# Isaac-McPadden/Farkle_II

Measured on AMD Instinct MI355X. Metric: simulated games/sec (whole node) at k=2, fixed strategy-grid size, higher is better.
Workload: dtype int32; 1 GPU; BASELINE configs[1]: k=2, 64-strategy grid, 10^7 games per GPU per step, root_seed 42, counts-only tallies; k=2, root_seed=42, parallelism=shuffle-range split x1, device=AMD Radeon Graphics, arch=gfx950:sramecc+:xnack-, compute_units=256, clock_mhz=2400

## Files before the change

farkle_ii_amd/csrc/fk_device.h:

```cpp
#pragma once

#include <hip/hip_runtime.h>
#include <stdint.h>

namespace fk {

constexpr uint32_t SS_INIT_A = 0x43b0d7e5u, SS_MULT_A = 0x931e8875u;
constexpr uint32_t SS_INIT_B = 0x8b51f9ddu, SS_MULT_B = 0x58f38dedu;
constexpr uint32_t SS_MIX_L = 0xca01f9ddu, SS_MIX_R = 0x4973f715u;

__host__ __device__ constexpr uint32_t ss_hc(int c) {
    uint32_t h = SS_INIT_A;
    for (int i = 0; i < c; ++i) h *= SS_MULT_A;
    return h;
}

__host__ __device__ inline uint32_t ss_hashmix(uint32_t v, uint32_t &hc) {
    v ^= hc;
    hc *= SS_MULT_A;
    v *= hc;
    v ^= v >> 16;
    return v;
}

// ... 765 lines not shown
    r.turn_score = farkle ? 0 : (r.turn_score + rr.score50);
    const bool hot = !farkle & sp.has(SF_AUTO_HOT) & (r.dice == 6u);
    if (LEAN) r.cB += hot ? 0x10000u : 0u;
    else r.cE += hot ? 1u : 0u;
    const bool keep = should_continue50(sp, r.turn_score, (int32_t)r.dice, (r.cE & BE_HAS_SCORED) != 0u, final_round, stb50, r.score);
    const bool over = farkle | (!hot & !keep);
    const uint32_t ts = over ? (uint32_t)r.turn_score : 0u;
    r.cE |= (ts >= 10u) ? BE_HAS_SCORED : 0u;
    const uint32_t banked = (r.cE & BE_HAS_SCORED) ? ts : 0u;
    r.score += (int32_t)banked;
    if (LEAN) r.cE += banked;
    r.cB = (banked > (r.cB & 0xffffu)) ? ((r.cB & 0xffff0000u) | banked) : r.cB;
    overflow = (r.turn_score > 1310) | ((r.cA & 0xffffu) > 64000u) | ((r.cC >> 16) > 63000u) | ((r.cD >> 16) > 63000u);
    return over;
}

typedef uint64_t lanes_t;
__host__ __device__ inline lanes_t lanes(bool p) {
#if defined(__HIP_DEVICE_COMPILE__)
    return __builtin_amdgcn_ballot_w64(p);
#else
    return p ? ~0ull : 0ull;
#endif
}
__host__ __device__ inline bool in_lanes(lanes_t m) {
#if defined(__HIP_DEVICE_COMPILE__)
    return __builtin_amdgcn_inverse_ballot_w64(m);
#else
    return m != 0ull;
#endif
}

template <uint32_t MIXED>
__host__ __device__ inline lanes_t flag_lanes(const Strat50 &s, uint32_t uniform_bits, uint32_t f) {
    return (f & MIXED) ? lanes((s.bits & f) != 0u) : ((uniform_bits & f) != 0u ? ~0ull : 0ull);
}

__host__ __device__ inline uint32_t pk_max_u16(uint32_t a, uint32_t b) {
#if defined(__HIP_DEVICE_COMPILE__)
    typedef unsigned short u16x2 __attribute__((ext_vector_type(2)));
    return __builtin_bit_cast(uint32_t, __builtin_elementwise_max(__builtin_bit_cast(u16x2, a), __builtin_bit_cast(u16x2, b)));
#else
    const uint32_t al = a & 0xffffu, bl = b & 0xffffu, ah = a >> 16, bh = b >> 16;
    return (al > bl ? al : bl) | ((ah > bh ? ah : bh) << 16);
#endif
}

template <bool LEAN, uint32_t MIXED>
__host__ __device__ inline bool roll_back_end50_core(int32_t score50, uint32_t used, uint32_t inc_c, uint32_t inc_d, uint32_t n, const Strat50 &sp,
                                                     uint32_t uniform_bits, bool final_round, int32_t stb50, RollRegs &r, bool &overflow) {
    const bool farkle = score50 == 0;
    r.cA += 1u + (farkle ? 0x10000u : 0u);
    r.cC += inc_c;
    r.cD += inc_d;
    r.dice = (used == n) ? 6u : (n - used);
    r.turn_score = farkle ? 0 : (r.turn_score + score50);
    const lanes_t farkle_l = lanes(score50 == 0);
    const lanes_t hot_l = ~farkle_l & flag_lanes<MIXED>(sp, uniform_bits, SF_AUTO_HOT) & lanes(r.dice == 6u);
    const bool hot = in_lanes(hot_l);
    if (LEAN) r.cB += hot ? 0x10000u : 0u;
    else r.cE += hot ? 1u : 0u;
    const lanes_t fr = lanes(final_round), above = lanes(r.score + r.turn_score > stb50);
    const lanes_t stop = fr & above & ~flag_lanes<MIXED>(sp, uniform_bits, SF_RUN_UP);
    const lanes_t force = fr & ~above;
    const lanes_t entry = lanes((r.cE & BE_HAS_SCORED) == 0u) & lanes(r.turn_score < 10);
    const lanes_t cs = flag_lanes<MIXED>(sp, uniform_bits, SF_CONSIDER_SCORE), cd = flag_lanes<MIXED>(sp, uniform_bits, SF_CONSIDER_DICE);
    const lanes_t ws = cs & lanes(r.turn_score < sp.thr50), wd = cd & lanes((int32_t)r.dice > sp.dice_thr());
    const lanes_t both = cs & cd & ~flag_lanes<MIXED>(sp, uniform_bits, SF_REQUIRE_BOTH);
    const lanes_t keep = ~stop & (force | entry | ((ws | wd) & (~both | (ws & wd))));
    const lanes_t over_l = farkle_l | (~hot_l & ~keep);
    const bool over = in_lanes(over_l), bank = in_lanes(over_l & ~entry);
    const uint32_t banked = bank ? (uint32_t)r.turn_score : 0u;
    r.cE |= bank ? BE_HAS_SCORED : 0u;
    r.score += (int32_t)banked;
    if (LEAN) r.cE += banked;
    r.cB = pk_max_u16(r.cB, banked);
    overflow = roll_overflow50(r);
    return over;
}

template <bool LEAN, uint32_t MIXED = 0xffffu>
__host__ __device__ inline bool roll_back_end50(uint32_t e, uint32_t choice, uint32_t n, const Strat50 &sp, uint32_t uniform_bits, bool final_round,
                                                int32_t stb50, RollRegs &r, bool &overflow) {
    const uint32_t d5 = choice & 3u, d1 = (choice >> 2) & 3u;
    const int32_t score50 = (int32_t)(e & 63u) - (int32_t)d5 - 2 * (int32_t)d1;
    const uint32_t used = ((e >> 6) & 7u) - d5 - d1;
    return roll_back_end50_core<LEAN, MIXED>(score50, used, (d5 << 16) + ((choice >> DCH_ANY5_SHIFT) & 1u), (d1 << 16) + ((choice >> DCH_ANY1_SHIFT) & 1u), n,
                                             sp, uniform_bits, final_round, stb50, r, overflow);
}

template <bool LEAN, uint32_t MIXED = 0xffffu>
__host__ __device__ inline bool roll_back_end50w(uint32_t e, uint32_t x, uint32_t n, const Strat50 &sp, uint32_t uniform_bits, bool final_round,
                                                 int32_t stb50, RollRegs &r, bool &overflow) {
    const int32_t score50 = (int32_t)(e & 63u) - (int32_t)((x >> DW_POINTS_SHIFT) & 0xffu);
    const uint32_t used = ((e >> 6) & 7u) - (x >> DW_DICE_SHIFT);
    return roll_back_end50_core<LEAN, MIXED>(score50, used, x & DW_INC, (x >> DW_D1_SHIFT) & DW_INC, n, sp, uniform_bits, final_round, stb50, r, overflow);
}

struct Table2 {
    uint32_t seat, rounds, trigger, final_round, safety;
    int32_t score_to_beat;
};
struct Advance2 {
    bool ended, sw;
};
__host__ __device__ inline Advance2 advance2_table50(bool over, int32_t score, int32_t target50, uint32_t max_rounds, Table2 &t) {
    const bool fr = t.final_round != 0u;
    const bool trig = over & !fr & (score >= target50);
    const bool close = over & !fr & !trig & (t.seat != 0u);
    const bool last = close & (t.rounds >= max_rounds);
    const bool ended = last | (over & fr);
    t.rounds += (close & !last) ? 1u : 0u;
    t.safety = last ? 1u : t.safety;
    t.score_to_beat = trig ? score : t.score_to_beat;
    t.trigger = trig ? t.seat : t.trigger;
    t.final_round = (fr | trig) ? 1u : 0u;
    const bool sw = over & !ended;
    t.seat ^= sw ? 1u : 0u;
    return Advance2{ended, sw};
}

constexpr uint32_t LEAN_IDX_SHIFT = 18;
struct LeanCounters {
    uint32_t cA, cB, cC, cD, cE;
};
struct Finish2 {
    bool completed;
    uint32_t winner, widx;
    uint32_t m[10];
};

__host__ __device__ inline Finish2 finish2_50_decoded(const LeanCounters &s0, const LeanCounters &s1, uint32_t rounds, uint32_t final_round,
                                                      uint32_t max_rounds) {
    const LeanCounters *seats[2] = {&s0, &s1};
    uint32_t score[2], idx[2], farkles[2], rolls[2], highest[2], sf_uses[2], sf_dice[2], so_uses[2], so_dice[2], hot[2];
    for (int s = 0; s < 2; ++s) {
        const LeanCounters &r = *seats[s];
        score[s] = r.cE & 0xffffu, idx[s] = r.cE >> LEAN_IDX_SHIFT;
        rolls[s] = r.cA & 0xffffu, farkles[s] = r.cA >> 16;
        highest[s] = r.cB & 0xffffu, hot[s] = r.cB >> 16;
        sf_uses[s] = r.cC & 0xffffu, sf_dice[s] = r.cC >> 16;
        so_uses[s] = r.cD & 0xffffu, so_dice[s] = r.cD >> 16;
    }
    Finish2 f;
    f.completed = max_rounds != 0u && final_round != 0u;
    f.winner = score[1] > score[0] ? 1u : 0u;
    const uint32_t w = f.winner;
    f.widx = idx[w];
    f.m[0] = score[w] * 50u, f.m[1] = rounds, f.m[2] = farkles[w], f.m[3] = rolls[w], f.m[4] = highest[w] * 50u;
    f.m[5] = sf_uses[w], f.m[6] = sf_dice[w], f.m[7] = so_uses[w], f.m[8] = so_dice[w], f.m[9] = hot[w];
    return f;
}

__host__ __device__ inline Finish2 finish2_50(const LeanCounters &s0, const LeanCounters &s1, uint32_t rounds, uint32_t final_round,
                                              uint32_t max_rounds) {
    (void)max_rounds;
    const bool second = (s1.cE & 0xffffu) > (s0.cE & 0xffffu);
    const uint32_t a = second ? s1.cA : s0.cA, b = second ? s1.cB : s0.cB, c = second ? s1.cC : s0.cC, d = second ? s1.cD : s0.cD,
                   e = second ? s1.cE : s0.cE;
    Finish2 f;
    f.completed = final_round != 0u;
    f.winner = second ? 1u : 0u;
    f.widx = e >> LEAN_IDX_SHIFT;
    f.m[0] = (e & 0xffffu) * 50u, f.m[1] = rounds, f.m[2] = a >> 16, f.m[3] = a & 0xffffu, f.m[4] = (b & 0xffffu) * 50u;
    f.m[5] = c & 0xffffu, f.m[6] = c >> 16, f.m[7] = d & 0xffffu, f.m[8] = d >> 16, f.m[9] = b >> 16;
    return f;
}

}
```

farkle_ii_amd/csrc/fk_kernels.h:

```cpp
#pragma once

#include "../../include/farkle_hip.h"
#include "fk_device.h"

#include <hip/hip_runtime.h>

#include <type_traits>

using namespace fk;

namespace {

constexpr uint32_t HC_AFTER_6_WORDS = ss_hc(24);
constexpr uint32_t HC_AFTER_12_WORDS = ss_hc(48);
constexpr uint32_t HC_AFTER_14_WORDS = ss_hc(56);

enum : uint32_t { MODE_PERM = 0, MODE_LIST = 1, MODE_BLOCKS = 2 };

enum : uint32_t {
    F_LO0 = 0, F_LO1, F_HI0, F_HI1, F_INC_LO0, F_INC_LO1, F_INC_HI0, F_INC_HI1,
    F_BUF, F_SCORE, F_CA, F_CB, F_CC, F_CD, F_CE, F_SPX, F_SPY, NF
};
constexpr uint32_t CE_HAS_BUF_SHIFT = 17, CE_HAS_SCORED = 1u << 16, CE_HAS_BUF = 1u << CE_HAS_BUF_SHIFT;
static_assert(CE_HAS_SCORED == BE_HAS_SCORED, "fk_device.h's roll back end sets the flag in cE");
// ... 934 lines not shown
            if (PK2) {
                const uint32_t *r0 = reinterpret_cast<const uint32_t *>(rec);
                rng.lo = (uint64_t)r0[0] | ((uint64_t)r0[1] << 32);
                rng.hi = (uint64_t)r0[2] | ((uint64_t)r0[3] << 32);
                rng.buf = r0[4];
            } else {
                rng.lo = (uint64_t)L(F_LO0, s) | ((uint64_t)L(F_LO1, s) << 32);
                rng.hi = (uint64_t)L(F_HI0, s) | ((uint64_t)L(F_HI1, s) << 32);
                rng.buf = L(F_BUF, s);
            }
            rng.has_buf = (cE & CE_HAS_BUF) ? 1u : 0u;
            key = 4u * roll_counts_sequential<3>(rng, n, nullptr);
        }
        rolls_this_turn += 1u;
        int32_t dthr = PK2 ? ((int32_t)own_bits >> 16) : (int32_t)(int8_t)(own_bits & 0xffu);
        asm volatile("" : "+v"(dthr));
        const Strat50 sp{own_thr, (own_bits & (0xffu | MIXED)) | (a.uflags & (0xff00u & ~MIXED)), dthr};
        uint32_t entry;
        const uint32_t choice = discard_lookup50w(a.score_lut, reinterpret_cast<const uint32_t *>(a.discard_lut + DISCARD_LUT_KEYS), key, (int32_t)n, turn_score, sp, entry);
        RollRegs rg{cA, cB, cC, cD, cE, score, dice, turn_score};
        bool overflow;
        const bool over = roll_back_end50w<LEAN, MIXED>(entry, choice, n, sp, a.uflags & (0xff00u & ~MIXED), final_round != 0u, score_to_beat, rg, overflow);
        cA = rg.cA, cB = rg.cB, cC = rg.cC, cD = rg.cD, cE = rg.cE, score = rg.score, dice = rg.dice, turn_score = rg.turn_score;
        const uint32_t guard = roll_guards50(rolls_before, rg);
        if (guard != RG_NONE) {
            raise(guard == RG_ROLL_LIMIT ? FK_ERR_ROLL_LIMIT : FK_ERR_COUNTER_OVERFLOW);
            return;
        }
        cE = (cE & ~CE_HAS_BUF) | (rng.has_buf << CE_HAS_BUF_SHIFT);
        if (GS) {
            if (over) {
                uint4 *g = reinterpret_cast<uint4 *>(G(s));
                g[0] = make_uint4((uint32_t)rng.lo, (uint32_t)(rng.lo >> 32), (uint32_t)rng.hi, (uint32_t)(rng.hi >> 32));
                g[1] = make_uint4(rng.buf, (uint32_t)score, cA, (cB & 0xffffu) | (own_turns << 16));
                uint32_t *g2 = reinterpret_cast<uint32_t *>(g + 2);
                g2[0] = cC;
                g2[1] = cD;
                g2[2] = (cB >> 16) | (cE & (CE_HAS_SCORED | CE_HAS_BUF));
                advance(score);
                return;
            }
        }
        if (LEAN) {
            rec[0] = make_uint2((uint32_t)rng.lo, (uint32_t)(rng.lo >> 32));
            rec[1] = make_uint2((uint32_t)rng.hi, (uint32_t)(rng.hi >> 32));
            rec[2] = make_uint2(rng.buf, cA);
            rec[3] = make_uint2(cB, cC);
            rec[4] = make_uint2(cD, cE);
        } else {
            L(F_LO0, s) = (uint32_t)rng.lo;
            L(F_LO1, s) = (uint32_t)(rng.lo >> 32);
            L(F_HI0, s) = (uint32_t)rng.hi;
            L(F_HI1, s) = (uint32_t)(rng.hi >> 32);
            L(F_BUF, s) = rng.buf;
            L(F_SCORE, s) = (uint32_t)score;
            L(F_CA, s) = cA;
            L(F_CB, s) = cB;
            L(F_CC, s) = cC;
            L(F_CD, s) = cD;
            L(F_CE, s) = cE;
        }
        if (PK2) advance2(over, score);
        else if (!GS && over) advance(score);
    };

    constexpr bool FLAT2 = PK2 && !BLK;
    static_assert(CE_IDX_SHIFT == LEAN_IDX_SHIFT, "finish2_50 reads the strategy index of a lean record");
    enum : uint32_t { HO_LDS_TALLY = 1, HO_REC0 = 2, HO_RECS = 4, HO_GS_OUT = 8, HO_OV = 16, HO_SCHED = 32, HO_PERM = 64, HO_IDX_STATE = 128,
                      HO_FLAT = 256 };
    typedef uint32_t u32x2 __attribute__((ext_vector_type(2)));
    typedef __attribute__((address_space(1))) u32x4 global_u4_rw;
    typedef const __attribute__((address_space(1))) u32x2 global_u2;
    typedef __attribute__((address_space(1))) uint32_t global_u32;
    uint32_t ho_bits = 0, st_rec = 0, ho_max_rounds = a.max_rounds, ho_thr = a.batch_threshold;
    int32_t ho_beat50 = a.beat50;
    uint64_t st_base = 0, inc_base = 0, idx_base = 0, sched_base = 0, strat_base = 0, rec0_base = 0;
    if constexpr (FLAT2) {
        const bool idx_state = a.state_dw == STATE_DW;
        const bool flat = !a.no_flat && (idx_state || a.seat_idx != nullptr) && (uint64_t)a.n_games * (2u * STATE_DW * 4u) <= 0xffffffffull;
        ho_bits = (a.use_lds_tally ? HO_LDS_TALLY : 0u) | (a.rec0 ? HO_REC0 : 0u) | (a.recs ? HO_RECS : 0u) | (a.gs_out ? HO_GS_OUT : 0u) |
             (a.n_ov ? HO_OV : 0u) | (a.sched ? HO_SCHED : 0u) | (a.mode == MODE_PERM ? HO_PERM : 0u) | (idx_state ? HO_IDX_STATE : 0u) |
             (flat ? HO_FLAT : 0u);
        st_rec = a.state_dw * 4u;
        st_base = (uint64_t)(uintptr_t)a.state, inc_base = (uint64_t)(uintptr_t)a.inc, sched_base = (uint64_t)(uintptr_t)a.sched;
        idx_base = idx_state ? st_base + R_IDX * 4u : (uint64_t)(uintptr_t)a.seat_idx;
        strat_base = (uint64_t)(uintptr_t)a.strat, rec0_base = (uint64_t)(uintptr_t)a.rec0;
        asm volatile("" : "+s"(ho_bits), "+s"(st_rec), "+s"(ho_max_rounds), "+s"(ho_thr), "+s"(ho_beat50), "+s"(st_base), "+s"(inc_base), "+s"(idx_base),
                     "+s"(sched_base), "+s"(strat_base), "+s"(rec0_base));
    }
    auto ld1 = [](uint64_t base, uint32_t off) __attribute__((always_inline)) -> uint32_t { return *(const global_u32 *)(base + (uint64_t)off); };
    auto ld2 = [](uint64_t base, uint32_t off) __attribute__((always_inline)) -> u32x2 { return *(global_u2 *)(base + (uint64_t)off); };
    auto ld4 = [](uint64_t base, uint32_t off) __attribute__((always_inline)) -> u32x4 { return *(global_u4 *)(base + (uint64_t)off); };

    auto init_game2 = [&](uint32_t ticket) __attribute__((always_inline)) {
        uint32_t ho = ho_bits;
        asm volatile("" : "+s"(ho));
        uint32_t id = ticket, slot = ticket;
        uint32_t id_ld = 0;
        if (ho & HO_SCHED) {
            id_ld = ld1(sched_base, ticket * 4u);
        } else if (ho & HO_PERM) {
            const uint32_t sh = id / a.gps, g = id - sh * a.gps;
            slot = g * a.n_sh + sh;
        }
        const uint32_t soff = slot * (2u * st_rec);
        const u32x4 s0 = ld4(st_base, soff), s1 = ld4(st_base, soff + st_rec);
        const u32x4 inc = ld4(inc_base, slot * 32u);
        const uint32_t ioff = (ho & HO_IDX_STATE) ? soff : slot * 4u;
        const uint32_t w0 = ld1(idx_base, ioff), w1 = ld1(idx_base, ioff + ((ho & HO_IDX_STATE) ? st_rec : 0u));
        if (ho & HO_SCHED) id = id_ld;
        const uint32_t idx0 = (ho & HO_IDX_STATE) ? w0 : (w0 & 0xffffu), idx1 = (ho & HO_IDX_STATE) ? w1 : (w1 >> 16);
        u32x2 pk0 = ld2(strat_base, idx0 * 8u), pk1 = ld2(strat_base, idx1 * 8u);
        game_id = id;
        seed_slot = slot;
        max_rounds = ho_max_rounds;
        if (ho & HO_OV) {
            uint32_t lo = 0, hi = a.n_ov;
            while (lo < hi) {
                const uint32_t mid = (lo + hi) >> 1;
                if (a.ov[mid].game < id) lo = mid + 1u;
                else hi = mid;
            }
            if (lo < a.n_ov && a.ov[lo].game == id) max_rounds = a.ov[lo].max_rounds;
        }
        uint2 *r0 = reinterpret_cast<uint2 *>(lds + lane_base), *r1 = reinterpret_cast<uint2 *>(lds + SEAT_STRIDE + lane_base);
        r0[0] = make_uint2(s0.x, s0.y), r0[1] = make_uint2(s0.z, s0.w);
        r0[2] = make_uint2(0u, 0u), r0[3] = make_uint2(0u, 0u), r0[4] = make_uint2(0u, idx0 << CE_IDX_SHIFT);
        r1[0] = make_uint2(s1.x, s1.y), r1[1] = make_uint2(s1.z, s1.w);
        r1[2] = make_uint2(0u, 0u), r1[3] = make_uint2(0u, 0u), r1[4] = make_uint2(0u, idx1 << CE_IDX_SHIFT);
        pk0.y = (pk0.y & 0xff00u) | ((uint32_t)(int32_t)(int8_t)(pk0.y & 0xffu) << 16);
        pk1.y = (pk1.y & 0xff00u) | ((uint32_t)(int32_t)(int8_t)(pk1.y & 0xffu) << 16);
        pk_seat0 = make_uint2(pk0.x, pk0.y);
        pk_delta = make_uint2(pk0.x ^ pk1.x, pk0.y ^ pk1.y);
        seat = 0;
        final_round = 0;
        score_to_beat = ho_beat50;
        own_inc_lo = (uint64_t)inc.x | ((uint64_t)inc.y << 32);
        own_inc_hi = (uint64_t)inc.z | ((uint64_t)inc.w << 32);
        own_thr = (int32_t)pk0.x;
        own_bits = pk0.y;
        own_rec = lds_addr(lane_base);
        own_inc_at = inc_base + (uint64_t)(slot * 32u);
        dice = 6;
        turn_score = 0;
        rolls_this_turn = 0;
        const bool none = max_rounds == 0u;
        rounds = none ? 0u : 1u;
        st = none ? (uint32_t)ST_ENDED : (uint32_t)ST_ACTIVE;
    };

    auto finish_game2 = [&]() __attribute__((always_inline)) {
        uint32_t ho = ho_bits;
        asm volatile("" : "+s"(ho));
        const uint2 *r0 = reinterpret_cast<const uint2 *>(lds + lane_base), *r1 = reinterpret_cast<const uint2 *>(lds + SEAT_STRIDE + lane_base);
        const uint2 p2 = r0[2], p3 = r0[3], p4 = r0[4], q2 = r1[2], q3 = r1[3], q4 = r1[4];
        const LeanCounters c0{p2.y, p3.x, p3.y, p4.x, p4.y}, c1{q2.y, q3.x, q3.y, q4.x, q4.y};
        const Finish2 f = finish2_50(c0, c1, rounds, final_round, max_rounds);
        const uint32_t idx0 = c0.cE >> CE_IDX_SHIFT, idx1 = c1.cE >> CE_IDX_SHIFT, widx = f.widx;
        if (ho & HO_GS_OUT) {
            const uint32_t last = (max_rounds != 0u && own_rec != lds_addr(lane_base)) ? 1u : 0u;
            const uint32_t t0 = rounds + ((final_round != 0u && last == 0u) ? 1u : 0u), t1 = rounds;
            const uint2 p0 = r0[0], p1 = r0[1], q0 = r1[0], q1 = r1[1];
            const uint32_t soff = seed_slot * (2u * st_rec);
            global_u4_rw *g0 = (global_u4_rw *)(st_base + (uint64_t)soff), *g1 = (global_u4_rw *)(st_base + (uint64_t)(soff + st_rec));
            g0[0] = u32x4{p0.x, p0.y, p1.x, p1.y};
            g0[1] = u32x4{p2.x, c0.cE & 0xffffu, c0.cA, (c0.cB & 0xffffu) | (t0 << 16)};
            g0[2] = u32x4{c0.cC, c0.cD, (c0.cB >> 16) | (c0.cE & (CE_HAS_SCORED | CE_HAS_BUF)), idx0};
            g1[0] = u32x4{q0.x, q0.y, q1.x, q1.y};
            g1[1] = u32x4{q2.x, c1.cE & 0xffffu, c1.cA, (c1.cB & 0xffffu) | (t1 << 16)};
            g1[2] = u32x4{c1.cC, c1.cD, (c1.cB >> 16) | (c1.cE & (CE_HAS_SCORED | CE_HAS_BUF)), idx1};
        }
        if (ho & HO_LDS_TALLY) {
            if (!f.completed || !(ho & HO_PERM)) {
                const uint32_t col = f.completed ? 1u : 2u;
                atomicAdd(&tl[idx0 * LT_COLS + col], 1ull);
                atomicAdd(&tl[idx1 * LT_COLS + col], 1ull);
            }
            if (f.completed) {
                unsigned long long *t = tl + widx * LT_COLS;
                atomicAdd(&t[0], 1ull);
#pragma unroll
                for (int j = 0; j < 10; ++j) {
                    atomicAdd(&t[3 + j], (unsigned long long)f.m[j]);
                    atomicAdd(&t[13 + j], (unsigned long long)f.m[j] * f.m[j]);
                }
            }
        }
        if (ho & HO_REC0) {
            const uint32_t d0 = f.completed ? (widx | (f.winner << 24)) : REC_SAFETY;
            *(global_u32 *)(rec0_base + (uint64_t)(game_id * 4u)) = d0;
            if (ho & HO_RECS) {
                uint32_t m[10];
#pragma unroll
                for (int j = 0; j < 10; ++j) m[j] = f.completed ? f.m[j] : 0u;
                uint4 *r = reinterpret_cast<uint4 *>(a.recs + (size_t)game_id * REC_DW);
                r[0] = make_uint4(d0, m[0], rounds | (m[2] << 16), m[3] | (m[4] << 16));
                r[1] = make_uint4(m[5] | (m[6] << 16), m[7] | (m[8] << 16), m[9], 0u);
            }
        }
    };

#ifdef FK_COUNT_HANDOVER
    uint32_t cnt_handovers = 0, cnt_served = 0, cnt_trips = 0, cnt_waiting = 0, cnt_rolling = 0;
#endif

    auto handover = [&](uint64_t waiting, auto flat) {
        constexpr bool FLAT = decltype(flat)::value;
        const bool mine = (st == ST_FRESH || st == ST_ENDED);
        if (st == ST_ENDED) {
            if constexpr (FLAT) finish_game2();
            else finish_game();
        }
        const uint32_t n = (uint32_t)__popcll(waiting);
        const uint32_t avail = pool_end - pool_next;
        uint32_t new_base = 0, new_avail = 0;
        if (avail < n && !exhausted) {
            const uint32_t first = (uint32_t)__builtin_amdgcn_readfirstlane(__ffsll((long long)waiting) - 1);
            uint32_t base = 0;
            if (mine && lane_id() == first) base = atomicAdd(a.ticket, TICKET_CHUNK);
            base = (uint32_t)__builtin_amdgcn_readlane((int)base, (int)first);
            if (base >= a.n_games) {
                exhausted = 1;
            } else {
                new_base = base;
                new_avail = min(TICKET_CHUNK, a.n_games - base);
                if (new_avail < TICKET_CHUNK) exhausted = 1;
            }
        }
        if (mine) {
            const uint32_t rank = mbcnt(waiting);
            uint32_t ticket = 0xffffffffu;
            if (rank < avail) ticket = pool_next + rank;
            else if (rank - avail < new_avail) ticket = new_base + (rank - avail);
            if (ticket != 0xffffffffu) {
                if constexpr (FLAT) init_game2(ticket);
                else init_game(a.sched ? a.sched[ticket] : ticket, ticket);
            } else {
                st = ST_DONE;
            }
        }
        if (n <= avail) {
            pool_next += n;
        } else {
            const uint32_t used_new = min(n - avail, new_avail);
            pool_next = new_base + used_new;
            pool_end = new_base + new_avail;
        }
    };

    auto handover_due = [&](uint64_t waiting, uint64_t active) -> bool {
        return waiting && (!active || (uint32_t)__popcll(waiting) >= ho_thr || exhausted);
    };
    auto play = [&](auto flat) {
        while (true) {
            uint64_t waiting = __ballot(st == ST_FRESH || st == ST_ENDED);
            uint64_t active = __ballot(st == ST_ACTIVE);
            if (!(waiting | active)) break;
            if (handover_due(waiting, active)) {
#ifdef FK_COUNT_HANDOVER
                cnt_handovers += 1u, cnt_served += (uint32_t)__popcll(waiting);
#endif
                handover(waiting, flat);
                continue;
            }
            bool playing = st == ST_ACTIVE;
            do {
#ifdef FK_COUNT_HANDOVER
                cnt_trips += 1u, cnt_waiting += (uint32_t)__popcll(waiting), cnt_rolling += (uint32_t)__popcll(active);
#endif
                if (playing) roll_step();
                playing = st == ST_ACTIVE;
                waiting = __ballot(st == ST_ENDED);
                active = __ballot(playing);
            } while (active && !handover_due(waiting, active));
        }
    };
    if constexpr (FLAT2) {
        if (ho_bits & HO_FLAT) play(std::true_type{});
        else play(std::false_type{});
    } else {
        play(std::false_type{});
    }

    if (a.use_lds_tally) {
        __syncthreads();
        for (uint32_t i = tid; i < a.S * LT_COLS; i += BLOCK) {
            const unsigned long long v = tl[i];
            if (v == 0ull) continue;
            const uint32_t idx = i / LT_COLS, c = i - idx * LT_COLS;
            if (c == LT_COLS - 1u) continue;
            const uint32_t col = (c == 0u) ? 0u : (c == 1u) ? 2u : (c == 2u) ? 3u : (c < 13u) ? (c + 1u) : (c + 2u);
            atomicAdd(&a.tally[(size_t)idx * FK_TALLY_COLS + col], v);
        }
    }
#ifdef FK_COUNT_HANDOVER
    if (a.hcount && lane_id() == 0u) {
        const uint32_t c[6] = {cnt_handovers, cnt_served, cnt_trips, cnt_waiting, cnt_rolling, 1u};
        for (int i = 0; i < 6; ++i) atomicAdd(&a.hcount[i], (unsigned long long)c[i]);
    }
#endif
    clock_stamp(a.clk, 1u);
}

#include "fk_play_hc.h"

constexpr uint32_t LAG_WIN_BIT = 0x8000u;

__global__ __launch_bounds__(256) void fk_lag_values_kernel(const uint32_t *recs, const uint16_t *perm_T, uint32_t perm_slots, uint32_t S,
                                                            uint32_t k, uint32_t gps, uint32_t n_games, uint16_t *V) {
    const size_t t = (size_t)blockIdx.x * blockDim.x + threadIdx.x;
    if (t >= (size_t)n_games * k) return;
    const uint32_t id = (uint32_t)(t / k), seat = (uint32_t)(t - (size_t)id * k);
    const uint32_t sh = id / gps, g = id - sh * gps;
    const uint4 q0 = *reinterpret_cast<const uint4 *>(recs + (size_t)id * REC_DW);
    const bool won = !(q0.x & REC_SAFETY) && ((q0.x >> 24) & 0x7fu) == seat;
    const uint32_t idx = perm_at(perm_T, S, perm_slots, sh, g * k + seat);
    V[(size_t)sh * S + idx] = (uint16_t)((q0.z & 0x7fffu) | (won ? LAG_WIN_BIT : 0u));
}

__global__ __launch_bounds__(256) void fk_lag_sums_kernel(const uint16_t *V, uint32_t S, uint32_t valid_from, uint32_t first_row, uint32_t n_rows,
                                                          uint32_t rows_per_seg, const int32_t *lags, uint32_t n_lags, long long *out) {
    const uint32_t s = blockIdx.x * blockDim.x + threadIdx.x;
    if (s >= S) return;
    const uint32_t r0 = first_row + blockIdx.y * rows_per_seg, r1 = min(r0 + rows_per_seg, n_rows);
    for (uint32_t li = 0; li < n_lags; ++li) {
        const uint32_t lag = (uint32_t)lags[li];
        long long n = 0, wx = 0, wy = 0, wxy = 0, rx = 0, ry = 0, rxx = 0, ryy = 0, rxy = 0;
        for (uint32_t r = max(r0, valid_from + lag); r < r1; ++r) {
            const uint32_t later = V[(size_t)r * S + s], earlier = V[(size_t)(r - lag) * S + s];
            const long long a = earlier & 0x7fffu, b = later & 0x7fffu, wa = earlier >> 15, wb = later >> 15;
            n += 1;
            wx += wa, wy += wb, wxy += wa & wb;
            rx += a, ry += b, rxx += a * a, ryy += b * b, rxy += a * b;
        }
        if (n == 0) continue;
        unsigned long long *o = reinterpret_cast<unsigned long long *>(out) + ((size_t)s * n_lags + li) * FK_LAG_COLS;
        const long long v[FK_LAG_COLS] = {n, wx, wy, wx, wy, wxy, rx, ry, rxx, ryy, rxy};
#pragma unroll
        for (int c = 0; c < FK_LAG_COLS; ++c)
            if (v[c]) atomicAdd(&o[c], (unsigned long long)v[c]);
    }
}


__device__ inline uint32_t walk_slot(uint32_t id, uint32_t gps, uint32_t n_sh, bool perm_mode) {
    if (!perm_mode) return id;
    const uint32_t sh = id / gps, g = id - sh * gps;
    return g * n_sh + sh;
}

constexpr uint32_t REDUCE_BLOCK = 1024, RT_COLS = 22;

__global__ __launch_bounds__(REDUCE_BLOCK) void fk_tally_reduce_kernel(const uint32_t *rec0, const uint32_t *recs, uint32_t n_games, uint32_t gps, uint32_t k,
                                                                       uint32_t S, const uint16_t *perm_T, uint32_t perm_slots,
                                                                       uint32_t sh_offset, uint32_t spb, uint32_t n_sh,
                                                                       uint32_t parts_per_batch, uint32_t slice, uint32_t first_batch,
                                                                       unsigned long long *tally) {
    extern __shared__ unsigned long long rt[];
    const uint32_t b_local = blockIdx.x / parts_per_batch, part = blockIdx.x - b_local * parts_per_batch;
    const uint32_t batch = first_batch + b_local;
    const uint64_t g_lo = (uint64_t)batch * spb, g_hi = g_lo + spb;
    const uint32_t sh_lo = g_lo > sh_offset ? (uint32_t)(g_lo - sh_offset) : 0u;
    const uint32_t sh_hi = (uint32_t)min<uint64_t>(n_sh, g_hi > sh_offset ? g_hi - sh_offset : 0u);
    if (sh_hi <= sh_lo) return;
    const uint32_t games = (sh_hi - sh_lo) * gps, per_part = (games + parts_per_batch - 1u) / parts_per_batch;
    const uint32_t first = sh_lo * gps + part * per_part, last = min(first + per_part, sh_lo * gps + games);
    const uint32_t s_lo = blockIdx.y * slice, s_n = min(slice, S - s_lo);
    for (uint32_t i = threadIdx.x; i < s_n * RT_COLS; i += REDUCE_BLOCK) rt[i] = 0ull;
    __syncthreads();
    constexpr uint32_t U = 4;
    for (uint32_t base = first + threadIdx.x; base < last; base += U * REDUCE_BLOCK) {
        uint32_t d0[U];
        uint4 q0[U], q1[U];
        bool mine[U];
#pragma unroll
        for (uint32_t u = 0; u < U; ++u) {
            const uint32_t id = base + u * REDUCE_BLOCK;
            d0[u] = id < last ? rec0[id] : REC_SAFETY - 1u;
        }
#pragma unroll
        for (uint32_t u = 0; u < U; ++u) {
            const uint32_t id = base + u * REDUCE_BLOCK;
            mine[u] = id < last && !(d0[u] & REC_SAFETY) && ((d0[u] & 0xffffffu) - s_lo) < s_n;
            if (mine[u]) {
                const uint4 *r = reinterpret_cast<const uint4 *>(recs + (size_t)id * REC_DW);
                q0[u] = r[0];
                q1[u] = r[1];
            }
        }
#pragma unroll
        for (uint32_t u = 0; u < U; ++u) {
            const uint32_t id = base + u * REDUCE_BLOCK;
            if (id < last && (d0[u] & REC_SAFETY)) {
                const uint32_t sh = id / gps, g = id - sh * gps;
                for (uint32_t s = 0; s < k; ++s) {
                    const uint32_t idx = perm_at(perm_T, S, perm_slots, sh, g * k + s) - s_lo;
                    if (idx < s_n) atomicAdd(&rt[idx * RT_COLS + 1u], 1ull);
                }
            }
            if (!mine[u]) continue;
            const uint32_t idx = (d0[u] & 0xffffffu) - s_lo;
            const unsigned long long m[10] = {q0[u].y, q0[u].z & 0xffffu, q0[u].z >> 16, q0[u].w & 0xffffu, q0[u].w >> 16,
                                              q1[u].x & 0xffffu, q1[u].x >> 16, q1[u].y & 0xffffu, q1[u].y >> 16, q1[u].z};
            unsigned long long *t = rt + idx * RT_COLS;
            atomicAdd(&t[0], 1ull);
#pragma unroll
            for (int j = 0; j < 10; ++j) {
                if (m[j]) {
                    atomicAdd(&t[2 + j], m[j]);
                    atomicAdd(&t[12 + j], m[j] * m[j]);
                }
            }
        }
    }
    __syncthreads();
    unsigned long long *out = tally + ((size_t)batch * S + s_lo) * FK_TALLY_COLS;
    for (uint32_t i = threadIdx.x; i < s_n * RT_COLS; i += REDUCE_BLOCK) {
        const unsigned long long v = rt[i];
        if (v == 0ull) continue;
        const uint32_t idx = i / RT_COLS, c = i - idx * RT_COLS;
        const uint32_t col = (c == 0u) ? 0u : (c == 1u) ? 3u : (c < 12u) ? (c + 2u) : (c + 3u);
        atomicAdd(&out[(size_t)idx * FK_TALLY_COLS + col], v);
    }
}

__global__ void fk_tally_direct_kernel(const uint32_t *recs, uint32_t n_games, uint32_t gps, uint32_t k, uint32_t S,
                                       const uint16_t *perm_T, uint32_t perm_slots, uint32_t sh_offset, uint32_t spb,
// ... 456 lines not shown
```

Measured before the change: 1.244 billion games/s.

## Trim finish-game LDS reads, narrow squares, and streamline flat handover loop

The finish path now reads only the two score words first, picks the winner, and loads that seat's counters alone; the full records of both seats are loaded only when game-state output is enabled. Squared tallies for the small 16-bit metrics use 32-bit multiplies instead of 64-bit ones. In flat mode the handover assigns tickets branch-free, falls straight into rolling instead of re-balloting, and stops forcing handovers after exhaustion once the local pool is empty. The aim is fewer LDS loads, cheaper arithmetic and fewer wave-wide ballots per loop trip. The risk is a behaviour difference in handover scheduling near pool exhaustion, and the narrowed squares assume the small metrics stay below 65536.

```diff
diff --git a/farkle_ii_amd/csrc/fk_device.h b/farkle_ii_amd/csrc/fk_device.h
--- a/farkle_ii_amd/csrc/fk_device.h
+++ b/farkle_ii_amd/csrc/fk_device.h
@@ -941,19 +941,30 @@
     return f;
 }
 
+__host__ __device__ inline bool finish2_second(uint32_t cE0, uint32_t cE1) { return (cE1 & 0xffffu) > (cE0 & 0xffffu); }
+
+__host__ __device__ inline Finish2 finish2_50_winner(const LeanCounters &w, bool second, uint32_t rounds, uint32_t final_round) {
+    Finish2 f;
+    f.completed = final_round != 0u;
+    f.winner = second ? 1u : 0u;
+    f.widx = w.cE >> LEAN_IDX_SHIFT;
+    f.m[0] = (w.cE & 0xffffu) * 50u, f.m[1] = rounds, f.m[2] = w.cA >> 16, f.m[3] = w.cA & 0xffffu, f.m[4] = (w.cB & 0xffffu) * 50u;
+    f.m[5] = w.cC & 0xffffu, f.m[6] = w.cC >> 16, f.m[7] = w.cD & 0xffffu, f.m[8] = w.cD >> 16, f.m[9] = w.cB >> 16;
+    return f;
+}
+
 __host__ __device__ inline Finish2 finish2_50(const LeanCounters &s0, const LeanCounters &s1, uint32_t rounds, uint32_t final_round,
                                               uint32_t max_rounds) {
     (void)max_rounds;
-    const bool second = (s1.cE & 0xffffu) > (s0.cE & 0xffffu);
-    const uint32_t a = second ? s1.cA : s0.cA, b = second ? s1.cB : s0.cB, c = second ? s1.cC : s0.cC, d = second ? s1.cD : s0.cD,
-                   e = second ? s1.cE : s0.cE;
-    Finish2 f;
-    f.completed = final_round != 0u;
-    f.winner = second ? 1u : 0u;
-    f.widx = e >> LEAN_IDX_SHIFT;
-    f.m[0] = (e & 0xffffu) * 50u, f.m[1] = rounds, f.m[2] = a >> 16, f.m[3] = a & 0xffffu, f.m[4] = (b & 0xffffu) * 50u;
-    f.m[5] = c & 0xffffu, f.m[6] = c >> 16, f.m[7] = d & 0xffffu, f.m[8] = d >> 16, f.m[9] = b >> 16;
-    return f;
-}
-
-}
+    const bool second = finish2_second(s0.cE, s1.cE);
+    return finish2_50_winner(second ? s1 : s0, second, rounds, final_round);
+}
+
+constexpr uint32_t FINISH2_POINT_METRICS = (1u << 0) | (1u << 4);
+__host__ __device__ inline uint64_t finish2_square(uint32_t j, uint32_t v) {
+    if ((FINISH2_POINT_METRICS >> j) & 1u) return (uint64_t)v * v;
+    const uint32_t x = v & 0xffffu;
+    return (uint64_t)(uint32_t)(x * x);
+}
+
+}
diff --git a/farkle_ii_amd/csrc/fk_kernels.h b/farkle_ii_amd/csrc/fk_kernels.h
--- a/farkle_ii_amd/csrc/fk_kernels.h
+++ b/farkle_ii_amd/csrc/fk_kernels.h
@@ -1110,15 +1110,19 @@
     auto finish_game2 = [&]() __attribute__((always_inline)) {
         uint32_t ho = ho_bits;
         asm volatile("" : "+s"(ho));
-        const uint2 *r0 = reinterpret_cast<const uint2 *>(lds + lane_base), *r1 = reinterpret_cast<const uint2 *>(lds + SEAT_STRIDE + lane_base);
-        const uint2 p2 = r0[2], p3 = r0[3], p4 = r0[4], q2 = r1[2], q3 = r1[3], q4 = r1[4];
-        const LeanCounters c0{p2.y, p3.x, p3.y, p4.x, p4.y}, c1{q2.y, q3.x, q3.y, q4.x, q4.y};
-        const Finish2 f = finish2_50(c0, c1, rounds, final_round, max_rounds);
-        const uint32_t idx0 = c0.cE >> CE_IDX_SHIFT, idx1 = c1.cE >> CE_IDX_SHIFT, widx = f.widx;
+        const uint32_t *w0 = lds + lane_base, *w1 = lds + SEAT_STRIDE + lane_base;
+        const uint32_t cE0 = w0[9], cE1 = w1[9];
+        const bool second = finish2_second(cE0, cE1);
+        const uint32_t *ww = second ? w1 : w0;
+        const LeanCounters cw{ww[5], ww[6], ww[7], ww[8], second ? cE1 : cE0};
+        const Finish2 f = finish2_50_winner(cw, second, rounds, final_round);
+        const uint32_t idx0 = cE0 >> CE_IDX_SHIFT, idx1 = cE1 >> CE_IDX_SHIFT, widx = f.widx;
         if (ho & HO_GS_OUT) {
             const uint32_t last = (max_rounds != 0u && own_rec != lds_addr(lane_base)) ? 1u : 0u;
             const uint32_t t0 = rounds + ((final_round != 0u && last == 0u) ? 1u : 0u), t1 = rounds;
-            const uint2 p0 = r0[0], p1 = r0[1], q0 = r1[0], q1 = r1[1];
+            const uint2 *r0 = reinterpret_cast<const uint2 *>(w0), *r1 = reinterpret_cast<const uint2 *>(w1);
+            const uint2 p0 = r0[0], p1 = r0[1], p2 = r0[2], p3 = r0[3], p4 = r0[4], q0 = r1[0], q1 = r1[1], q2 = r1[2], q3 = r1[3], q4 = r1[4];
+            const LeanCounters c0{p2.y, p3.x, p3.y, p4.x, p4.y}, c1{q2.y, q3.x, q3.y, q4.x, q4.y};
             const uint32_t soff = seed_slot * (2u * st_rec);
             global_u4_rw *g0 = (global_u4_rw *)(st_base + (uint64_t)soff), *g1 = (global_u4_rw *)(st_base + (uint64_t)(soff + st_rec));
             g0[0] = u32x4{p0.x, p0.y, p1.x, p1.y};
@@ -1140,7 +1144,7 @@
 #pragma unroll
                 for (int j = 0; j < 10; ++j) {
                     atomicAdd(&t[3 + j], (unsigned long long)f.m[j]);
-                    atomicAdd(&t[13 + j], (unsigned long long)f.m[j] * f.m[j]);
+                    atomicAdd(&t[13 + j], (unsigned long long)finish2_square((uint32_t)j, f.m[j]));
                 }
             }
         }
@@ -1185,14 +1189,19 @@
                 if (new_avail < TICKET_CHUNK) exhausted = 1;
             }
         }
-        if (mine) {
+        if constexpr (FLAT) {
+            const uint32_t rank = mbcnt(waiting);
+            uint32_t ticket = rank < avail ? pool_next + rank : (rank - avail < new_avail) ? new_base + (rank - avail) : 0xffffffffu;
+            ticket = mine ? ticket : 0xffffffffu;
+            st = (mine && ticket == 0xffffffffu) ? (uint32_t)ST_DONE : st;
+            if (ticket != 0xffffffffu) init_game2(ticket);
+        } else if (mine) {
             const uint32_t rank = mbcnt(waiting);
             uint32_t ticket = 0xffffffffu;
             if (rank < avail) ticket = pool_next + rank;
             else if (rank - avail < new_avail) ticket = new_base + (rank - avail);
             if (ticket != 0xffffffffu) {
-                if constexpr (FLAT) init_game2(ticket);
-                else init_game(a.sched ? a.sched[ticket] : ticket, ticket);
+                init_game(a.sched ? a.sched[ticket] : ticket, ticket);
             } else {
                 st = ST_DONE;
             }
@@ -1206,20 +1215,27 @@
         }
     };
 
-    auto handover_due = [&](uint64_t waiting, uint64_t active) -> bool {
+    auto handover_due_general = [&](uint64_t waiting, uint64_t active) -> bool {
         return waiting && (!active || (uint32_t)__popcll(waiting) >= ho_thr || exhausted);
+    };
+    auto handover_due = [&](uint64_t waiting, uint64_t active, auto flat) -> bool {
+        if constexpr (!decltype(flat)::value) return handover_due_general(waiting, active);
+        else return waiting && (!active || (uint32_t)__popcll(waiting) >= ho_thr || (exhausted && pool_next != pool_end));
     };
     auto play = [&](auto flat) {
         while (true) {
             uint64_t waiting = __ballot(st == ST_FRESH || st == ST_ENDED);
             uint64_t active = __ballot(st == ST_ACTIVE);
             if (!(waiting | active)) break;
-            if (handover_due(waiting, active)) {
+            if (handover_due(waiting, active, flat)) {
 #ifdef FK_COUNT_HANDOVER
                 cnt_handovers += 1u, cnt_served += (uint32_t)__popcll(waiting);
 #endif
                 handover(waiting, flat);
-                continue;
+                if constexpr (!decltype(flat)::value) continue;
+#ifdef FK_COUNT_HANDOVER
+                waiting = __ballot(st == ST_FRESH || st == ST_ENDED), active = __ballot(st == ST_ACTIVE);
+#endif
             }
             bool playing = st == ST_ACTIVE;
             do {
@@ -1230,7 +1246,7 @@
                 playing = st == ST_ACTIVE;
                 waiting = __ballot(st == ST_ENDED);
                 active = __ballot(playing);
-            } while (active && !handover_due(waiting, active));
+            } while (active && !handover_due(waiting, active, flat));
         }
     };
     if constexpr (FLAT2) {
```

New measurement: 1.264 billion games/s (median of 6 runs). 1.02x the previous value.
